# yekaizhou/duet

Hardware: AMD Instinct MI355X
Metric: SV support-read marks clustered+phased /sec; bit-exact phased_sv.vcf vs ref (higher is better)
Workload: dtype u32/u64 integer + f64 threshold compares; 1 GPU; BASELINE configs[1]: synthetic 1 contig, 1001116 SV marks / 100000 candidates / 159991 tagged reads, resident in HBM; step = ef_classify + ef_finalize_own, two launches (phasing, E/F; ef_seed_sort 0: ; marks_per_gpu=1001116, candidates_per_gpu=100000, reads_per_gpu=159991, parallelism=contig-sharded x1, svlen_thres=50, suppread_thres=2, device_preheat_steps=2700

## Files before the change

### duet_amd/csrc/duet_ef.hip

```cpp

#include <hip/hip_runtime.h>
#include <hip/hip_ext.h>
#include <stdint.h>
#include <stdio.h>
#include <stdlib.h>
#include <string.h>
#include <string>
#include <vector>

#include "duet_ef.h"
#include "duet_internal.h"

#pragma clang fp contract(off)

namespace {

#ifdef DUET_STAMPS
#define STAMP(k, i) do { if (threadIdx.x == 0 && p.stamps) p.stamps[((size_t)(k) * 65536 + blockIdx.x) * 8 + (i)] = wall_clock64(); } while (0)
#else
#define STAMP(k, i) do { } while (0)
#endif

#include "duet_seeds.hip.h"

// ... 1397 lines not shown
            uint32_t any = 0;
            for (uint32_t k = k0; k <= k1; ++k) any |= (p.n_one[k] == 0) ? 1u : 0u;
            const uint32_t n0 = p.n_one[k0], base = p.ctg_off[k0] + k0 + 1;
            const bool lds_mode = k0 == k1 && n0 > 0 && n0 <= kOneLds;
            if (lds_mode)
                for (uint32_t i = tid; i < n0; i += 256u) s_one[i] = p.onebuf[base + i];
            __syncthreads();
#pragma unroll
            for (int r = 0; r < TPB; ++r) {
                const uint32_t cc = g0 + 256u * r + tid;
                if (cc < n_cands) finalize_candidate(p, cc, codes[r], pss[r], k0, lds_mode, s_one, n0, any);
            }
            __syncthreads();
            continue;
        }
        const uint32_t c0 = tile * 256u;
        const uint32_t c = c0 + tid;
        const bool live = c < n_cands;
        const uint8_t code = live ? p.out_pred[c] : 0;
        const uint32_t ps_in = live ? p.out_ps[c] : 0;
        if (tid == 0) {
            const uint32_t last = min(c0 + 255u, n_cands - 1);
            const uint32_t k0 = (DYN && p.cand_contig) ? (uint32_t)p.cand_contig[c0] : p.blk_ctg[tile];
            uint32_t k1 = k0;
            while (last >= p.ctg_off[k1 + 1]) ++k1;
            uint32_t any = 0;
            for (uint32_t k = k0; k <= k1; ++k) any |= (p.n_one[k] == 0);
            const uint32_t n0 = p.n_one[k0];
            s_meta[0] = k0;
            s_meta[1] = (k0 == k1 && n0 > 0 && n0 <= kOneLds) ? n0 : kEmpty;
            s_meta[2] = any;
            s_meta[3] = p.ctg_off[k0] + k0 + 1;
        }
        __syncthreads();
        STAMP(2, 1);
        const uint32_t k0 = s_meta[0], n_lds = s_meta[1], any_empty = s_meta[2];
        const bool lds_mode = n_lds != kEmpty;
        if (lds_mode) {
            const uint32_t *src = p.onebuf + s_meta[3];
            for (uint32_t i = tid; i < n_lds; i += 256u) s_one[i] = src[i];
            __syncthreads();
        }
        STAMP(2, 2);
        if (live) finalize_candidate(p, c, code, ps_in, k0, lds_mode, s_one, n_lds, any_empty);
        if (!DYN) break;
        __syncthreads();
    }
}

constexpr uint32_t kOwnMaxTiles = 2048;
constexpr uint32_t kOwnTab = 2048;
constexpr uint32_t kOwnKeys = 1024;

struct OwnArgs {
    TileRecs recs;
    const uint64_t *seed_ent, *read_tag;
    const uint32_t *cand_pos, *cand_off, *cand_svread, *cand_refread, *mark_read, *c2rec;
    uint32_t *out_ps, *status;
    uint8_t *out_pred;
    uint32_t c_lo, c_hi;
};

template <class F>
__device__ __forceinline__ void own_each_entry(TileRecs recs, const uint64_t *seed_ent, uint32_t c_lo, uint32_t c_hi, uint32_t first,
                                               uint32_t stride, F f)
{
    const uint32_t b_lo = c_lo / kCandPerBlock, b_hi = (c_hi - 1) / kCandPerBlock;
    for (uint32_t b = b_lo + first; b <= b_hi; b += stride) {
        const ulonglong4 rec = recs[b];
        const uint32_t cnt = (uint32_t)rec.x;
        for (uint32_t j = 0; j < cnt; ++j) {
            const uint64_t e = j == 0 ? rec.y : (j == 1 ? rec.z : (j == 2 ? rec.w : seed_ent[(size_t)b * kCandPerBlock + j]));
            const uint32_t c = (uint32_t)(e >> 32);
            if (c >= c_lo && c < c_hi) f((uint32_t)e);
        }
    }
}

__device__ __forceinline__ uint32_t own_nearest_walk(const OwnArgs &a, uint32_t pos)
{
    uint32_t best = 0;
    int64_t bd = -1;
    own_each_entry(a.recs, a.seed_ent, a.c_lo, a.c_hi, 0u, 1u, [&](uint32_t ps) {
        const int64_t d = llabs((int64_t)pos - (int64_t)ps);
        if (bd < 0 || d < bd || (d == bd && ps > best)) { bd = d; best = ps; }
    });
    return best;
}
__device__ __forceinline__ bool own_member_walk(const OwnArgs &a, uint32_t key)
{
    bool hit = false;
    own_each_entry(a.recs, a.seed_ent, a.c_lo, a.c_hi, 0u, 1u, [&](uint32_t ps) { hit = hit || ps == key; });
    return hit;
}

template <class F>
__device__ __forceinline__ void own_each_tag(const OwnArgs &a, uint32_t b, uint32_t e, F f)
{
    for (uint32_t m = b; m < e; ++m) {
        const uint32_t r = a.mark_read[m];
        f(r == kEmpty ? kUntagged : a.read_tag[r]);
    }
}

__device__ __forceinline__ void finalize_candidate_walk(const OwnArgs &a, uint32_t c, uint32_t code, uint32_t ps_in)
{
    if (code & kDivZero) {
        atomicOr(&a.status[0], 1u);
        a.out_pred[c] = 0;
        a.out_ps[c] = 0;
        return;
    }
    const uint32_t c_pos = a.cand_pos[c];
    if (code & (kClass2 | kClass2Slow)) {
        Vote v = {0, 0, 0, 0, 0, 0};
        uint32_t ps = 0;
        const uint32_t mb = a.cand_off[c], me = a.cand_off[c + 1];
        if (code & kClass2) {
            const uint32_t *rec = a.c2rec + (size_t)ps_in * kC2Words;
            v.allhap = rec[0];
            const uint32_t ng = rec[1];
            uint32_t best = 0;
            for (uint32_t k = 0; k < (uint32_t)kC2Groups; ++k) {
                const uint32_t *g = rec + 2 + 6 * k;
                if (k < ng && g[1] > best && own_member_walk(a, g[0])) {
                    best = g[1];
                    ps = g[0];
                    v.hap1 = g[2]; v.hap2 = g[3];
                    v.t1 = g[4]; v.t2 = g[5];
                    v.hap0 = v.allhap - v.hap1 - v.hap2;
                }
            }
        } else {
            uint32_t best = 0;
            own_each_tag(a, mb, me, [&](uint64_t t) {
                if (t != kUntagged && tag_pc(t) <= kPcMax) ++v.allhap;
            });
            uint32_t done_ps = kEmpty;
            own_each_tag(a, mb, me, [&](uint64_t t) {
                if (t == kUntagged || tag_pc(t) > kPcMax) return;
                const uint32_t g = tag_ps(t);
                if (g == done_ps || (g == ps && best)) return;
                if (!own_member_walk(a, g)) return;
                uint32_t n = 0, n1 = 0, n2 = 0;
                uint64_t s1 = 0, s2 = 0;
                own_each_tag(a, mb, me, [&](uint64_t u) {
                    if (u == kUntagged || tag_pc(u) > kPcMax || tag_ps(u) != g) return;
                    ++n;
                    const uint32_t hap = tag_hap(u), pc = tag_pc(u);
                    n1 += hap == 1 ? 1u : 0u; s1 += hap == 1 ? pc : 0u;
                    n2 += hap == 2 ? 1u : 0u; s2 += hap == 2 ? pc : 0u;
                });
                done_ps = g;
                if (n > best) {
                    best = n; ps = g;
                    v.hap1 = n1; v.hap2 = n2; v.t1 = s1; v.t2 = s2;
                    v.hap0 = v.allhap - n1 - n2;
                }
            });
        }
        if (v.hap1 == 0 && v.hap2 == 0) ps = own_nearest_walk(a, c_pos);
        a.out_pred[c] = (uint8_t)decide(2, v, me - mb, a.cand_svread[c], a.cand_refread[c]);
        a.out_ps[c] = ps;
        return;
    }
    a.out_pred[c] = (uint8_t)(code & 3u);
    a.out_ps[c] = own_nearest_walk(a, c_pos);
}

__device__ __forceinline__ uint32_t wave_max_u32(uint32_t v)
{
    v = max(v, (uint32_t)__builtin_amdgcn_update_dpp(0, (int)v, 0xB1, 0xF, 0xF, false));
    v = max(v, (uint32_t)__builtin_amdgcn_update_dpp(0, (int)v, 0x4E, 0xF, 0xF, false));
    v = max(v, (uint32_t)__builtin_amdgcn_update_dpp(0, (int)v, 0x124, 0xF, 0xF, false));
    v = max(v, (uint32_t)__builtin_amdgcn_update_dpp(0, (int)v, 0x128, 0xF, 0xF, false));
    v = max(v, (uint32_t)__builtin_amdgcn_update_dpp(0, (int)v, 0x142, 0xA, 0xF, false));
    v = max(v, (uint32_t)__builtin_amdgcn_update_dpp(0, (int)v, 0x143, 0xC, 0xF, false));
    return (uint32_t)__builtin_amdgcn_readlane((int)v, 63);
}

__device__ __forceinline__ void own_sort_set(const uint32_t *s_tab, uint32_t *s_key, uint32_t *s_one, uint32_t *s_part, uint32_t u)
{
    const uint32_t tid = threadIdx.x, lane = tid & 63u, wave = tid >> 6;
    uint32_t mv[kOwnTab / 256u], cnt = 0;
#pragma unroll
    for (uint32_t j = 0; j < kOwnTab / 256u; ++j) {
        mv[j] = s_tab[tid + 256u * j];
        cnt += mv[j] != kEmpty ? 1u : 0u;
    }
    uint32_t x = cnt;
#pragma unroll
    for (int d = 1; d < 64; d <<= 1) {
        const uint32_t y = __shfl_up(x, d, 64);
        if ((int)lane >= d) x += y;
    }
    if (lane == 63) s_part[wave] = x;
    __syncthreads();
    uint32_t at = x - cnt;
#pragma unroll
    for (uint32_t w = 0; w < 4; ++w) at += w < wave ? s_part[w] : 0u;
#pragma unroll
    for (uint32_t j = 0; j < kOwnTab / 256u; ++j)
        if (mv[j] != kEmpty) s_key[at++] = mv[j];
    const uint32_t U = (u + 63u) & ~63u, nblk = U >> 6;
    if (tid < U - u) s_key[u + tid] = kEmpty;
    __syncthreads();
    for (uint32_t b = wave; b < nblk; b += 4u) s_key[b * 64u + lane] = wave_sort64(s_key[b * 64u + lane], lane);
    __syncthreads();
    for (uint32_t i = tid; i < U; i += 256u) {
        const uint32_t me = s_key[i];
        uint32_t rank = 0;
        for (uint32_t b = 0; b < nblk; b += 4u) {
            const uint32_t *b0 = s_key + b * 64u, *b1 = s_key + min(b + 1u, nblk - 1u) * 64u;
            const uint32_t *b2 = s_key + min(b + 2u, nblk - 1u) * 64u, *b3 = s_key + min(b + 3u, nblk - 1u) * 64u;
            uint32_t p0 = 0, p1 = 0, p2 = 0, p3 = 0;
#pragma unroll
            for (uint32_t st = 32; st > 0; st >>= 1) {
                p0 += b0[p0 + st - 1u] < me ? st : 0u;
                p1 += b1[p1 + st - 1u] < me ? st : 0u;
                p2 += b2[p2 + st - 1u] < me ? st : 0u;
                p3 += b3[p3 + st - 1u] < me ? st : 0u;
            }
            p0 += b0[p0] < me ? 1u : 0u;
            p1 += b1[p1] < me ? 1u : 0u;
            p2 += b2[p2] < me ? 1u : 0u;
            p3 += b3[p3] < me ? 1u : 0u;
            rank += p0 + (b + 1u < nblk ? p1 : 0u) + (b + 2u < nblk ? p2 : 0u) + (b + 3u < nblk ? p3 : 0u);
        }
        if (me != kEmpty) s_one[rank] = me;
    }
    __syncthreads();
}

__device__ __forceinline__ void own_vote_from_marks(const uint32_t *mark_read, const uint64_t *read_tag, uint32_t mb, uint32_t me_,
                                                 const uint32_t *s_tab, Vote *vo, uint32_t *pso)
{
    auto each = [&](auto f) {
        for (uint32_t m0 = mb; m0 < me_; m0 += 8) {
            uint32_t r[8];
            uint64_t t[8];
#pragma unroll
            for (int j = 0; j < 8; ++j) r[j] = mark_read[m0 + j < me_ ? m0 + j : mb];
#pragma unroll
            for (int j = 0; j < 8; ++j) t[j] = read_tag[r[j] == kEmpty ? 0u : r[j]];
#pragma unroll
            for (int j = 0; j < 8; ++j)
                if (m0 + j < me_) f(r[j] == kEmpty ? kUntagged : t[j]);
        }
    };
    auto member = [&](uint32_t key) -> bool {
        uint32_t h = (key * 2654435761u) >> (32u - 11u);
        for (;;) {
            const uint32_t v = s_tab[h];
            if (v == key) return true;
            if (v == kEmpty) return false;
            h = (h + 1u) & (kOwnTab - 1u);
        }
    };
    Vote v = {0, 0, 0, 0, 0, 0};
    uint32_t ps = 0, best = 0, done_ps = kEmpty;
    each([&](uint64_t t) {
        if (t != kUntagged && tag_pc(t) <= kPcMax) ++v.allhap;
    });
    each([&](uint64_t t) {
        if (t == kUntagged || tag_pc(t) > kPcMax) return;
        const uint32_t g = tag_ps(t);
        if (g == done_ps || (g == ps && best)) return;
        if (!member(g)) return;
        uint32_t n = 0, n1 = 0, n2 = 0;
        uint64_t s1 = 0, s2 = 0;
        each([&](uint64_t u) {
            if (u == kUntagged || tag_pc(u) > kPcMax || tag_ps(u) != g) return;
            ++n;
            const uint32_t hap = tag_hap(u), pc = tag_pc(u);
            n1 += hap == 1 ? 1u : 0u; s1 += hap == 1 ? pc : 0u;
            n2 += hap == 2 ? 1u : 0u; s2 += hap == 2 ? pc : 0u;
        });
        done_ps = g;
        if (n > best) {
            best = n; ps = g;
            v.hap1 = n1; v.hap2 = n2; v.t1 = s1; v.t2 = s2;
            v.hap0 = v.allhap - n1 - n2;
        }
    });
    *vo = v;
    *pso = ps;
}

__device__ __forceinline__ bool own_probe(uint32_t *s_tab, uint32_t key, uint32_t h)
{
    for (uint32_t probes = 0; probes < kOwnTab; ++probes) {
        const uint32_t old = atomicCAS(&s_tab[h], kEmpty, key);
        if (old == kEmpty) return true;
        if (old == key) return false;
        h = (h + 1u) & (kOwnTab - 1u);
    }
    return false;
}

constexpr uint32_t kOwnWin = 64;

__global__ __launch_bounds__(256) void ef_finalize_own(const Params p)
{
    __shared__ uint32_t s_tab[kOwnTab];
    __shared__ uint32_t s_key[kOwnKeys];
    __shared__ uint32_t s_one[kOwnKeys];
    __shared__ uint32_t s_win[kOwnWin];
    __shared__ uint32_t s_mm[4][2];
    __shared__ uint32_t s_red[4][3];
    __shared__ uint32_t s_part[4];
    __shared__ uint32_t s_nwin;
    __shared__ __align__(8) uint32_t s_c2[kC2Quota * kC2Words];
    const uint32_t tid = threadIdx.x, lane = tid & 63u, wave = tid >> 6;
    STAMP(2, 0);
    if (blockIdx.x == 0 && tid == 0) p.status[1] = 0;
    const uint32_t n_cands = p.C;
    const uint32_t nK = p.n_small;
    auto coff = [&](uint32_t kk) -> uint32_t { return p.ctg_small[kk]; };
    const uint32_t tile = blockIdx.x;
    const uint32_t c0 = tile * 256u, c = c0 + tid;
    const bool live = c < n_cands;
    const uint32_t cl = live ? c : n_cands - 1u;
    const uint32_t last = min(c0 + 255u, n_cands - 1);
    const uint32_t keys_cap = (p.dbg & DUET_DBG_EF_OWN_SMALLTAB) ? 8u : kOwnKeys;
    const uint32_t win_cap = (p.dbg & DUET_DBG_EF_OWN_SMALLTAB) ? 2u : kOwnWin;
    const TileRecs recs{reinterpret_cast<const ulonglong4 *>(p.blk_rec)};
    constexpr uint32_t kPre = 2;
    static_assert(kPre == 2, "the overflow loop selects between rec[0] and rec[1]");
    ulonglong4 rec[kPre], ext[kPre];
    auto load_recs = [&](uint32_t b_lo, uint32_t b_hi) {
#pragma unroll
        for (uint32_t i = 0; i < kPre; ++i) {
            const uint32_t b = min(b_lo + tid + 256u * i, b_hi);
            rec[i] = recs[b];
            ext[i] = recs.second(b);
        }
    };
    const uint32_t code_ld = p.out_pred[cl], ps_ld = p.out_ps[cl], pos_ld = p.cand_pos[cl];
    const uint32_t o0_ld = p.cand_off[cl], o1_ld = p.cand_off[cl + 1u];
    const uint32_t sv_ld = p.cand_svread[cl], rf_ld = p.cand_refread[cl];
    constexpr uint32_t kPairs = kC2Quota * kC2Words / 2;
    const uint2 *c2src = reinterpret_cast<const uint2 *>(p.c2rec + (size_t)tile * kC2Quota * kC2Words);
    const uint2 a0 = c2src[tid], a1 = c2src[tid + 256u < kPairs ? tid + 256u : tid];
    uint32_t lo = 0, hi = nK;
    while (hi - lo > 1) {
        const uint32_t mid = (lo + hi) >> 1;
        if (coff(mid) <= c0) lo = mid; else hi = mid;
    }
    uint32_t k_first = lo;
    while (k_first < nK && coff(k_first) == coff(k_first + 1)) ++k_first;
    {
        const uint32_t kf = k_first < nK ? k_first : 0u;
        load_recs(coff(kf) / kCandPerBlock, (coff(kf + 1) - 1) / kCandPerBlock);
    }
    asm volatile("" ::"v"(code_ld), "v"(ps_ld), "v"(pos_ld), "v"(o0_ld), "v"(o1_ld), "v"(sv_ld), "v"(rf_ld), "v"(a0.x), "v"(a0.y),
                 "v"(a1.x), "v"(a1.y));
    {
        uint2 *dst = reinterpret_cast<uint2 *>(s_c2);
        dst[tid] = a0;
        if (tid + 256u < kPairs) dst[tid + 256u] = a1;
    }
    const uint32_t code = live ? code_ld : 0u, ps_in = live ? ps_ld : 0u, c_pos = live ? pos_ld : 0u;
    const uint32_t c_o0 = live ? o0_ld : 0u, c_o1 = live ? o1_ld : 0u;
    const uint32_t c_svread = live ? sv_ld : 0u, c_refread = live ? rf_ld : 0u;
    for (uint32_t k = lo; k < nK && coff(k) <= last; ++k) {
        const uint32_t c_lo = coff(k), c_hi = coff(k + 1);
        if (c_lo == c_hi) continue;
        const uint32_t b_lo = c_lo / kCandPerBlock, b_hi = (c_hi - 1) / kCandPerBlock;
        if (k != k_first) load_recs(b_lo, b_hi);
#pragma unroll
        for (uint32_t i = 0; i < kOwnTab / 256u; ++i) s_tab[tid + 256u * i] = kEmpty;
        if (tid == 0) s_nwin = 0;
        const bool mine = live && c >= c_lo && c < c_hi;
        const bool asks = mine && code >= 4u && !(code & kDivZero);
        {
            const uint32_t mn = wave_max_u32(asks ? ~c_pos : 0u), mx = wave_max_u32(asks ? c_pos + 1u : 0u);
            if (lane == 0) { s_mm[wave][0] = mn; s_mm[wave][1] = mx; }
        }
        lds_barrier();
        STAMP(2, 1);
        asm volatile("" ::"v"(rec[0].x), "v"(rec[1].x), "v"(rec[0].y), "v"(rec[1].y), "v"(rec[0].z), "v"(rec[1].z), "v"(rec[0].w),
                     "v"(rec[1].w), "v"(ext[0].x), "v"(ext[1].x), "v"(ext[0].y), "v"(ext[1].y), "v"(ext[0].z), "v"(ext[1].z),
                     "v"(ext[0].w), "v"(ext[1].w));
        uint32_t pmin, pmax;
        {
            const uint32_t a0 = max(max(s_mm[0][0], s_mm[1][0]), max(s_mm[2][0], s_mm[3][0]));
            const uint32_t a1 = max(max(s_mm[0][1], s_mm[1][1]), max(s_mm[2][1], s_mm[3][1]));
            pmin = a1 ? ~a0 : 0u;
            pmax = a1 ? a1 - 1u : 0u;
        }
        uint32_t fresh = 0, leftp = 0, rinv = 0;
        static_assert(kOwnTab == 1u << 11, "the hash takes 11 bits");
        auto slot_of = [](uint32_t key) -> uint32_t { return (key * 2654435761u) >> (32u - 11u); };
        auto count_new = [&](bool nw, uint32_t key) {
            fresh += nw ? 1u : 0u;
            leftp = max(leftp, (nw && key <= pmin) ? key + 1u : 0u);
            rinv = max(rinv, (nw && key >= pmax) ? ~key : 0u);
            if (nw && key > pmin && key < pmax) {
                const uint32_t at = atomicAdd(&s_nwin, 1u);
                if (at < kOwnWin) s_win[at] = key;
            }
        };
        auto insert = [&](uint64_t e) {
            const uint32_t cc = (uint32_t)(e >> 32), key = (uint32_t)e;
            if (cc >= c_lo && cc < c_hi) count_new(own_probe(s_tab, key, slot_of(key)), key);
        };
        uint32_t coll = 0;
        auto group = [&](const uint64_t (&e)[4], uint32_t first, uint32_t n_in, uint32_t cnt, uint32_t bit0) {
            uint32_t key[4], old[4];
            bool ok[4];
#pragma unroll
            for (uint32_t j = 0; j < 4; ++j) {
                const uint32_t cc = (uint32_t)(e[j] >> 32);
                key[j] = (uint32_t)e[j];
                ok[j] = j < n_in && first + j < cnt && cc >= c_lo && cc < c_hi;
                old[j] = kEmpty;
            }
#pragma unroll
            for (uint32_t j = 0; j < 4; ++j)
                if (ok[j]) old[j] = atomicCAS(&s_tab[slot_of(key[j])], kEmpty, key[j]);
#pragma unroll
            for (uint32_t j = 0; j < 4; ++j) {
                coll |= (ok[j] && old[j] != kEmpty && old[j] != key[j]) ? 1u << (bit0 + j) : 0u;
                count_new(ok[j] && old[j] == kEmpty, key[j]);
            }
        };
#pragma unroll
        for (uint32_t i = 0; i < kPre; ++i) {
            const uint32_t cnt = b_lo + tid + 256u * i <= b_hi ? (uint32_t)rec[i].x : 0u;
            if (__any(cnt > 0u)) {
                const uint64_t e[4] = {rec[i].y, rec[i].z, rec[i].w, 0ull};
                group(e, 0u, 3u, cnt, 7u * i);
            }
            if (__any(cnt > 3u)) {
                const uint64_t e[4] = {ext[i].x, ext[i].y, ext[i].z, ext[i].w};
                group(e, 3u, 4u, cnt, 7u * i + 3u);
            }
        }
        while (coll) {
            const uint32_t j = (uint32_t)__ffs(coll) - 1u;
            coll &= coll - 1u;
            uint32_t key = 0;
#pragma unroll
            for (uint32_t i = 0; i < kPre; ++i) {
                key = j == 7u * i + 0u ? (uint32_t)rec[i].y : key;
                key = j == 7u * i + 1u ? (uint32_t)rec[i].z : key;
                key = j == 7u * i + 2u ? (uint32_t)rec[i].w : key;
                key = j == 7u * i + 3u ? (uint32_t)ext[i].x : key;
                key = j == 7u * i + 4u ? (uint32_t)ext[i].y : key;
                key = j == 7u * i + 5u ? (uint32_t)ext[i].z : key;
                key = j == 7u * i + 6u ? (uint32_t)ext[i].w : key;
            }
            count_new(own_probe(s_tab, key, (slot_of(key) + 1u) & (kOwnTab - 1u)), key);
        }
        auto overflow = [&](uint32_t b, uint32_t cnt, uint32_t from) {
            constexpr uint32_t kLong = 24;
            if (cnt > from && cnt <= kLong) {
                const uint64_t *ov = p.seed_ent + (size_t)b * kCandPerBlock;
#pragma unroll 1
                for (uint32_t j = from; j < cnt; j += 4) {
                    uint64_t e[4];
#pragma unroll
                    for (uint32_t t = 0; t < 4; ++t) e[t] = ov[min(j + t, cnt - 1u)];
#pragma unroll
                    for (uint32_t t = 0; t < 4; ++t)
                        if (j + t < cnt) insert(e[t]);
                }
            }
            unsigned long long todo = __ballot(cnt > kLong);
            while (todo) {
                const uint32_t h = (uint32_t)__ffsll((long long)todo) - 1u;
                todo &= todo - 1ull;
                const uint32_t b_h = (uint32_t)__builtin_amdgcn_readlane((int)b, h), cnt_h = (uint32_t)__builtin_amdgcn_readlane((int)cnt, h);
                const uint64_t *ov = p.seed_ent + (size_t)b_h * kCandPerBlock;
                for (uint32_t j = from + lane; j < cnt_h; j += 64u) insert(ov[j]);
            }
        };
#pragma unroll 1
        for (uint32_t i = 0, b0 = b_lo; b0 <= b_hi; ++i, b0 += 256u) {
            const uint32_t b = b0 + tid;
            uint32_t cnt, from = 7u;
            if (i < kPre) {
                cnt = b <= b_hi ? (uint32_t)(i == 0 ? rec[0].x : rec[1].x) : 0u;
            } else {
                ulonglong4 r = {0, 0, 0, 0};
                if (b <= b_hi) r = recs[b];
                cnt = (uint32_t)r.x;
                if (cnt > 0) insert(r.y);
                if (cnt > 1) insert(r.z);
                if (cnt > 2) insert(r.w);
                from = 3u;
            }
            overflow(b, cnt, from);
        }
        {
            const uint32_t l = wave_max_u32(leftp), r = wave_max_u32(rinv), o = wave_sum(fresh);
            if (lane == 0) { s_red[wave][0] = l; s_red[wave][1] = r; s_red[wave][2] = o; }
        }
        lds_barrier();
        STAMP(2, 2);
        const uint32_t u = s_red[0][2] + s_red[1][2] + s_red[2][2] + s_red[3][2];
        const uint32_t Lp = max(max(s_red[0][0], s_red[1][0]), max(s_red[2][0], s_red[3][0]));
        const uint32_t Ri = max(max(s_red[0][1], s_red[1][1]), max(s_red[2][1], s_red[3][1]));
        const uint32_t n_win = s_nwin;
        const bool over = u > keys_cap;
        const bool sorted = !over && n_win > win_cap;
        if (sorted) own_sort_set(s_tab, s_key, s_one, s_part, u);
        STAMP(2, 5);
        auto nearest = [&](uint32_t pos) -> uint32_t {
            if (sorted) return nearest_seed(s_one, u, pos);
            uint32_t best = 0;
            int64_t bd = -1;
            auto look = [&](uint32_t v) {
                const int64_t d = llabs((int64_t)pos - (int64_t)v);
                if (bd < 0 || d < bd || (d == bd && v > best)) { bd = d; best = v; }
            };
            if (Lp) look(Lp - 1u);
            if (Ri) look(~Ri);
            for (uint32_t i = 0; i < n_win; ++i) look(s_win[i]);
            return best;
        };
        auto member = [&](uint32_t key) -> bool {
            uint32_t h = (key * 2654435761u) >> (32u - 11u);
            for (;;) {
                const uint32_t v = s_tab[h];
                if (v == key) return true;
                if (v == kEmpty) return false;
                h = (h + 1u) & (kOwnTab - 1u);
            }
        };
        if (mine) {
            if (u == 0) {
                if (code != 0) p.out_pred[c] = 0;
                if (ps_in != 0) p.out_ps[c] = 0;
            } else if (code >= 4u) {
                if (code & kDivZero) {
                    atomicOr(&p.status[0], 1u);
                    p.out_pred[c] = 0;
                    p.out_ps[c] = 0;
                } else if (over) {
                    const OwnArgs a = {recs, p.seed_ent, p.read_tag, p.cand_pos, p.cand_off, p.cand_svread, p.cand_refread, p.mark_read, p.c2rec,
                                       p.out_ps, p.status, p.out_pred, c_lo, c_hi};
                    finalize_candidate_walk(a, c, code, ps_in);
                } else if (code & kClass2Slow) {
                    Vote v;
                    uint32_t ps;
                    own_vote_from_marks(p.mark_read, p.read_tag, c_o0, c_o1, s_tab, &v, &ps);
                    if (v.hap1 == 0 && v.hap2 == 0) ps = nearest(c_pos);
                    p.out_pred[c] = (uint8_t)decide(2, v, c_o1 - c_o0, c_svread, c_refread);
                    p.out_ps[c] = ps;
                } else if (code & kClass2) {
                    uint32_t w[kC2Words];
                    const uint32_t own0 = tile * kC2Quota;
                    if (ps_in >= own0 && ps_in < own0 + kC2Quota) {
#pragma unroll
                        for (int i = 0; i < kC2Words; ++i) w[i] = s_c2[(ps_in - own0) * kC2Words + i];
                    } else {
                        const uint32_t *rec2 = p.c2rec + (size_t)ps_in * kC2Words;
#pragma unroll
                        for (int i = 0; i < kC2Words; ++i) w[i] = rec2[i];
                    }
                    Vote v = {0, 0, 0, 0, 0, 0};
                    uint32_t ps = 0, best = 0;
                    v.allhap = w[0];
                    const uint32_t ng = w[1];
#pragma unroll
                    for (int g = 0; g < kC2Groups; ++g) {
                        if ((uint32_t)g < ng && w[2 + 6 * g + 1] > best && member(w[2 + 6 * g])) {
                            best = w[2 + 6 * g + 1];
                            ps = w[2 + 6 * g];
                            v.hap1 = w[2 + 6 * g + 2]; v.hap2 = w[2 + 6 * g + 3];
                            v.t1 = w[2 + 6 * g + 4]; v.t2 = w[2 + 6 * g + 5];
                            v.hap0 = v.allhap - v.hap1 - v.hap2;
                        }
                    }
                    if (v.hap1 == 0 && v.hap2 == 0) ps = nearest(c_pos);
                    p.out_pred[c] = (uint8_t)decide(2, v, c_o1 - c_o0, c_svread, c_refread);
                    p.out_ps[c] = ps;
                } else {
                    p.out_pred[c] = (uint8_t)(code & 3u);
                    p.out_ps[c] = nearest(c_pos);
                }
            }
        }
        STAMP(2, 6);
        __syncthreads();
    }
}

__global__ void plan_mark_starts(const uint32_t *ctg_off, uint32_t K, uint8_t *ctg_start)
{
    const uint32_t k = blockIdx.x * blockDim.x + threadIdx.x;
    if (k < K && ctg_off[k] < ctg_off[k + 1]) ctg_start[ctg_off[k]] = 1;
}

__global__ void plan_device(const uint32_t *ctg_off, uint32_t K, uint32_t B, uint32_t *ctg_off_copy, uint32_t *n_one_and_status,
                            uint32_t *blk_ctg)
{
    const uint32_t b = blockIdx.x * blockDim.x + threadIdx.x;
    if (b <= K) ctg_off_copy[b] = ctg_off[b];
    if (b < K + 8) n_one_and_status[b] = 0;
    if (b >= B) return;
    const uint32_t c = b * kCandPerBlock;
    uint32_t lo = 0, hi = K;
    while (hi - lo > 1) {
        const uint32_t mid = (lo + hi) >> 1;
        if (ctg_off[mid] <= c) lo = mid; else hi = mid;
    }
    blk_ctg[b] = lo;
}

__global__ void plan_device_contigs(const uint16_t *cand_contig, const uint32_t *n_cands, uint32_t K, uint32_t B,
                                    uint32_t *ctg_off_copy, uint32_t *n_one_and_status, uint32_t *blk_ctg)
{
    const uint32_t t = blockIdx.x * blockDim.x + threadIdx.x;
    const uint32_t N = *n_cands;
    if (t <= K) {
        uint32_t lo = 0, hi = N;
        while (lo < hi) {
            const uint32_t mid = lo + ((hi - lo) >> 1);
            if (cand_contig[mid] < t) lo = mid + 1; else hi = mid;
        }
        ctg_off_copy[t] = t == K ? N : lo;
    }
    if (t < K + 8) n_one_and_status[t] = 0;
    if (t < B) {
        const uint32_t c = t * kCandPerBlock;
        blk_ctg[t] = c < N ? (uint32_t)cand_contig[c] : 0u;
    }
}


}

thread_local std::string duet_g_last_error;

namespace {

inline int fail(duet_ctx *ctx, int code, const std::string &msg) { return duet_fail(ctx, code, msg); }
inline int reserve(duet_ctx *ctx, DevBuf &b, size_t bytes) { return duet_reserve(ctx, b, bytes); }

size_t c2_slots(uint32_t B, uint32_t C) { return (size_t)B * kC2Quota + (C / 8u > 256u ? C / 8u : 256u); }

int ensure_plan(duet_ctx *ctx, const duet_ef_problem *pr, hipStream_t stream)
{
    const uint32_t K = pr->n_contigs, C = pr->n_cands;
    if (ctx->plan_C == C && ctx->plan_off.size() == (size_t)K + 1 && ctx->plan_stream == stream &&
        memcmp(ctx->plan_off.data(), pr->cand_ctg_off, sizeof(uint32_t) * (K + 1)) == 0)
        return DUET_OK;
    const uint32_t B = (C + kCandPerBlock - 1) / kCandPerBlock;
    const size_t small_words = (size_t)(K + 1) + K + 8 + (size_t)B + 16 + (size_t)B * 16;
    const size_t want[6] = {small_words * 4, C, (size_t)B * kCandPerBlock * 8, ((size_t)C + K + 1) * 4, ((size_t)C + K + 1) * 4,
                            c2_slots(B, C) * kC2Words * 4};
    DevBuf *bufs[6] = {&ctx->ws_small, &ctx->ws_start, &ctx->ws_ent, &ctx->ws_one, &ctx->ws_tmp, &ctx->ws_c2};
    bool grow = ctx->plan_stream != stream;
    for (int i = 0; i < 6; ++i) grow = grow || want[i] > bufs[i]->cap;
    const size_t stage_bytes = ((size_t)K + 1 + B) * 4;
    grow = grow || stage_bytes > ctx->plan_stage_cap;
    int rc;
    if (grow) {
        HIP_TRY(ctx, hipDeviceSynchronize());
        for (int i = 0; i < 6; ++i)
            if ((rc = reserve(ctx, *bufs[i], want[i]))) return rc;
        if (stage_bytes > ctx->plan_stage_cap) {
            if (ctx->plan_stage) HIP_TRY(ctx, hipHostFree(ctx->plan_stage));
            ctx->plan_stage = nullptr;
            ctx->plan_stage_cap = 0;
            HIP_TRY(ctx, hipHostMalloc((void **)&ctx->plan_stage, stage_bytes + stage_bytes / 4 + 4096, hipHostMallocDefault));
            ctx->plan_stage_cap = stage_bytes + stage_bytes / 4 + 4096;
        }
    } else {
        HIP_TRY(ctx, hipEventSynchronize(ctx->plan_ev));
    }
    uint32_t *w = (uint32_t *)ctx->ws_small.ptr;
    ctx->d_ctg_off = w;            w += K + 1;
    ctx->d_n_one = w;              w += K;
    ctx->d_status = w;             w += 8;
    ctx->d_blk_ctg = w;            w += B;
    w += ((uintptr_t)w & 63) ? (64 - ((uintptr_t)w & 63)) / 4 : 0;
    ctx->d_blk_cnt = w;
    uint32_t *h_off = ctx->plan_stage, *h_blk = ctx->plan_stage + (K + 1);
    memcpy(h_off, pr->cand_ctg_off, sizeof(uint32_t) * (K + 1));
    {
        uint32_t k = 0;
        for (uint32_t b = 0; b < B; ++b) {
            const uint32_t c = b * kCandPerBlock;
            while (c >= pr->cand_ctg_off[k + 1]) ++k;
            h_blk[b] = k;
        }
    }
    HIP_TRY(ctx, hipMemcpyAsync(ctx->d_ctg_off, h_off, sizeof(uint32_t) * (K + 1), hipMemcpyHostToDevice, stream));
    if (B) HIP_TRY(ctx, hipMemcpyAsync(ctx->d_blk_ctg, h_blk, sizeof(uint32_t) * B, hipMemcpyHostToDevice, stream));
    HIP_TRY(ctx, hipEventRecord(ctx->plan_ev, stream));
    HIP_TRY(ctx, hipMemsetAsync(ctx->d_n_one, 0, sizeof(uint32_t) * ((size_t)K + 8), stream));
    if (C) HIP_TRY(ctx, hipMemsetAsync(ctx->ws_start.ptr, 0, C, stream));
    hipLaunchKernelGGL(plan_mark_starts, dim3((K + 255) / 256), dim3(256), 0, stream, ctx->d_ctg_off, K,
                       (uint8_t *)ctx->ws_start.ptr);
    HIP_TRY(ctx, hipGetLastError());
    ctx->ef_seeds_stale = false;
    ctx->plan_off.assign(pr->cand_ctg_off, pr->cand_ctg_off + K + 1);
    ctx->plan_C = C;
    ctx->plan_stream = stream;
    return DUET_OK;
}

int validate(duet_ctx *ctx, const duet_ef_problem *pr, const void *out_pred, const void *out_ps)
{
    if (!ctx) return fail(nullptr, DUET_ERR_INVALID, "null context");
    if (!pr) return fail(ctx, DUET_ERR_INVALID, "null problem");
    if (!pr->cand_ctg_off) return fail(ctx, DUET_ERR_INVALID, "cand_ctg_off is null");
    if (pr->n_contigs == 0 && pr->n_cands != 0) return fail(ctx, DUET_ERR_INVALID, "candidates without contigs");
    if (pr->cand_ctg_off[0] != 0 || pr->cand_ctg_off[pr->n_contigs] != pr->n_cands)
        return fail(ctx, DUET_ERR_INVALID, "cand_ctg_off must start at 0 and end at n_cands");
    for (uint32_t k = 0; k < pr->n_contigs; ++k)
        if (pr->cand_ctg_off[k] > pr->cand_ctg_off[k + 1])
            return fail(ctx, DUET_ERR_INVALID, "cand_ctg_off must be non-decreasing");
    if (pr->n_cands) {
        if (!pr->cand_pos || !pr->cand_svlen || !pr->cand_svread || !pr->cand_refread || !pr->cand_gt_ok ||
            !pr->cand_off || !pr->mark_read || !out_pred || !out_ps)
            return fail(ctx, DUET_ERR_INVALID, "null array");
        if (pr->n_reads && !pr->read_tag) return fail(ctx, DUET_ERR_INVALID, "read_tag is null");
    }
    return DUET_OK;
}

}

extern "C" {

int duet_abi_version(void) { return DUET_ABI_VERSION; }

const char *duet_last_error(const duet_ctx *ctx) { return ctx ? ctx->err.c_str() : duet_g_last_error.c_str(); }

duet_ctx *duet_ctx_create(int device_id)
{
    int n = 0;
    hipError_t e = hipGetDeviceCount(&n);
    if (e != hipSuccess || n <= 0) {
        duet_g_last_error = std::string("no HIP device: ") + (e != hipSuccess ? hipGetErrorString(e) : "device count is 0");
        return nullptr;
    }
    if (device_id < 0 || device_id >= n) {
        duet_g_last_error = "device id out of range";
        return nullptr;
    }
    if ((e = hipSetDevice(device_id)) != hipSuccess) {
        duet_g_last_error = std::string("hipSetDevice: ") + hipGetErrorString(e);
        return nullptr;
    }
    hipDeviceProp_t prop;
    if ((e = hipGetDeviceProperties(&prop, device_id)) != hipSuccess) {
        duet_g_last_error = std::string("hipGetDeviceProperties: ") + hipGetErrorString(e);
        return nullptr;
    }
    if (strncmp(prop.gcnArchName, "gfx950", 6) != 0) {
        duet_g_last_error = std::string("device is ") + prop.gcnArchName + ", this library is built for gfx950 only";
// ... 404 lines not shown
```

Measured before the change: 63.72 billion marks/s.

## Batch hash-table inserts in finalize_own and aggregate window appends per wave

The kernel now issues all preloaded entries' LDS atomicCAS inserts in one unrolled batch. Non-owned entries go to a per-lane dummy slot instead of being branched around. The left/right boundary bookkeeping becomes min reductions rather than per-entry count_new calls. Per-lane atomicAdd on the window counter is replaced by a wave-level ballot prefix sum with a single atomic per wave, and collision reprobing is skipped unless some lane saw a foreign key. The aim is to cut divergent control flow and LDS atomic contention, at the cost of more registers for the key/old arrays and a slightly larger shared table.

Result: no change. 63.69 billion marks/s, median of 4 (-0.0%).

```diff
diff --git a/duet_amd/csrc/duet_ef.hip b/duet_amd/csrc/duet_ef.hip
--- a/duet_amd/csrc/duet_ef.hip
+++ b/duet_amd/csrc/duet_ef.hip
@@ -1723,7 +1723,7 @@
 
 __global__ __launch_bounds__(256) void ef_finalize_own(const Params p)
 {
-    __shared__ uint32_t s_tab[kOwnTab];
+    __shared__ uint32_t s_tab[kOwnTab + 64];
     __shared__ uint32_t s_key[kOwnKeys];
     __shared__ uint32_t s_one[kOwnKeys];
     __shared__ uint32_t s_win[kOwnWin];
@@ -1791,6 +1791,7 @@
         if (k != k_first) load_recs(b_lo, b_hi);
 #pragma unroll
         for (uint32_t i = 0; i < kOwnTab / 256u; ++i) s_tab[tid + 256u * i] = kEmpty;
+        if (tid < 64u) s_tab[kOwnTab + tid] = kEmpty;
         if (tid == 0) s_nwin = 0;
         const bool mine = live && c >= c_lo && c < c_hi;
         const bool asks = mine && code >= 4u && !(code & kDivZero);
@@ -1803,6 +1804,7 @@
         asm volatile("" ::"v"(rec[0].x), "v"(rec[1].x), "v"(rec[0].y), "v"(rec[1].y), "v"(rec[0].z), "v"(rec[1].z), "v"(rec[0].w),
                      "v"(rec[1].w), "v"(ext[0].x), "v"(ext[1].x), "v"(ext[0].y), "v"(ext[1].y), "v"(ext[0].z), "v"(ext[1].z),
                      "v"(ext[0].w), "v"(ext[1].w));
+        STAMP(2, 3);
         uint32_t pmin, pmax;
         {
             const uint32_t a0 = max(max(s_mm[0][0], s_mm[1][0]), max(s_mm[2][0], s_mm[3][0]));
@@ -1826,53 +1828,89 @@
             const uint32_t cc = (uint32_t)(e >> 32), key = (uint32_t)e;
             if (cc >= c_lo && cc < c_hi) count_new(own_probe(s_tab, key, slot_of(key)), key);
         };
-        uint32_t coll = 0;
-        auto group = [&](const uint64_t (&e)[4], uint32_t first, uint32_t n_in, uint32_t cnt, uint32_t bit0) {
-            uint32_t key[4], old[4];
-            bool ok[4];
-#pragma unroll
-            for (uint32_t j = 0; j < 4; ++j) {
-                const uint32_t cc = (uint32_t)(e[j] >> 32);
-                key[j] = (uint32_t)e[j];
-                ok[j] = j < n_in && first + j < cnt && cc >= c_lo && cc < c_hi;
-                old[j] = kEmpty;
-            }
-#pragma unroll
-            for (uint32_t j = 0; j < 4; ++j)
-                if (ok[j]) old[j] = atomicCAS(&s_tab[slot_of(key[j])], kEmpty, key[j]);
-#pragma unroll
-            for (uint32_t j = 0; j < 4; ++j) {
-                coll |= (ok[j] && old[j] != kEmpty && old[j] != key[j]) ? 1u << (bit0 + j) : 0u;
-                count_new(ok[j] && old[j] == kEmpty, key[j]);
-            }
-        };
+        constexpr uint32_t kEnt = 7u * kPre;
+        const uint32_t n_c = c_hi - c_lo;
+        uint32_t key[kEnt], old[kEnt], left_d = kEmpty, right_d = kEmpty;
+        bool take[kEnt];
 #pragma unroll
         for (uint32_t i = 0; i < kPre; ++i) {
             const uint32_t cnt = b_lo + tid + 256u * i <= b_hi ? (uint32_t)rec[i].x : 0u;
-            if (__any(cnt > 0u)) {
-                const uint64_t e[4] = {rec[i].y, rec[i].z, rec[i].w, 0ull};
-                group(e, 0u, 3u, cnt, 7u * i);
-            }
-            if (__any(cnt > 3u)) {
-                const uint64_t e[4] = {ext[i].x, ext[i].y, ext[i].z, ext[i].w};
-                group(e, 3u, 4u, cnt, 7u * i + 3u);
-            }
-        }
-        while (coll) {
-            const uint32_t j = (uint32_t)__ffs(coll) - 1u;
-            coll &= coll - 1u;
-            uint32_t key = 0;
-#pragma unroll
-            for (uint32_t i = 0; i < kPre; ++i) {
-                key = j == 7u * i + 0u ? (uint32_t)rec[i].y : key;
-                key = j == 7u * i + 1u ? (uint32_t)rec[i].z : key;
-                key = j == 7u * i + 2u ? (uint32_t)rec[i].w : key;
-                key = j == 7u * i + 3u ? (uint32_t)ext[i].x : key;
-                key = j == 7u * i + 4u ? (uint32_t)ext[i].y : key;
-                key = j == 7u * i + 5u ? (uint32_t)ext[i].z : key;
-                key = j == 7u * i + 6u ? (uint32_t)ext[i].w : key;
-            }
-            count_new(own_probe(s_tab, key, (slot_of(key) + 1u) & (kOwnTab - 1u)), key);
+#pragma unroll
+            for (uint32_t j = 0; j < 7; ++j) take[7 * i + j] = __any(cnt > (j < 3u ? 0u : j));
+        }
+        asm volatile("" ::"v"(pmin), "v"(pmax));
+#pragma unroll
+        for (uint32_t i = 0; i < kPre; ++i) {
+            const uint32_t cnt = b_lo + tid + 256u * i <= b_hi ? (uint32_t)rec[i].x : 0u;
+            const uint64_t e[7] = {rec[i].y, rec[i].z, rec[i].w, ext[i].x, ext[i].y, ext[i].z, ext[i].w};
+#pragma unroll
+            for (uint32_t j = 0; j < 7; ++j) {
+                const uint32_t n = 7 * i + j;
+                key[n] = kEmpty;
+                old[n] = kEmpty;
+                if (!take[n]) continue;
+                const bool ok = (j < cnt) & ((uint32_t)(e[j] >> 32) - c_lo < n_c);
+                key[n] = ok ? (uint32_t)e[j] : kEmpty;
+                uint32_t slot = slot_of((uint32_t)e[j]);
+                asm volatile("" : "+v"(slot));
+                old[n] = atomicCAS(&s_tab[ok ? slot : kOwnTab + lane], kEmpty, key[n]);
+                left_d = min(left_d, pmin - key[n]);
+                right_d = min(right_d, key[n] - pmax);
+            }
+        }
+        leftp = max(leftp, left_d <= pmin ? pmin - left_d + 1u : 0u);
+        rinv = max(rinv, right_d <= 0xFFFFFFFEu - pmax ? ~(pmax + right_d) : 0u);
+        const uint32_t width = pmax > pmin ? pmax - pmin - 1u : 0u;
+        uint32_t inwin = 0;
+        uint32_t met_other = 0;
+#pragma unroll
+        for (uint32_t n = 0; n < kEnt; ++n) {
+            if (!take[n]) continue;
+            const bool won = old[n] == kEmpty;
+            const uint32_t mine_new = won ? key[n] : kEmpty;
+            fresh += mine_new != kEmpty ? 1u : 0u;
+            inwin |= mine_new - pmin - 1u < width ? 1u << n : 0u;
+            met_other |= (won ? key[n] : old[n]) ^ key[n];
+        }
+#ifdef DUET_STAMPS
+        asm volatile("" ::"v"(inwin), "v"(met_other), "v"(fresh));
+#endif
+        STAMP(2, 4);
+        if (__builtin_amdgcn_ballot_w64(met_other != 0u) != 0) {
+            uint32_t coll = 0;
+#pragma unroll
+            for (uint32_t n = 0; n < kEnt; ++n)
+                coll |= ((old[n] != kEmpty) & (old[n] != key[n])) ? 1u << n : 0u;
+            while (coll) {
+                const uint32_t j = (uint32_t)__ffs(coll) - 1u;
+                coll &= coll - 1u;
+                uint32_t k1 = 0;
+#pragma unroll
+                for (uint32_t n = 0; n < kEnt; ++n) k1 = j == n ? key[n] : k1;
+                const bool nw = own_probe(s_tab, k1, (slot_of(k1) + 1u) & (kOwnTab - 1u));
+                fresh += nw ? 1u : 0u;
+                inwin |= (nw && k1 > pmin && k1 < pmax) ? 1u << j : 0u;
+            }
+        }
+        if (__builtin_amdgcn_ballot_w64(inwin != 0u) != 0) {
+            const uint32_t mine_n = (uint32_t)__popc(inwin);
+            uint32_t before = 0, total = 0;
+#pragma unroll
+            for (uint32_t b = 0; b < 4; ++b) {
+                const uint64_t m = __builtin_amdgcn_ballot_w64(((mine_n >> b) & 1u) != 0u);
+                before += __builtin_amdgcn_mbcnt_hi((uint32_t)(m >> 32), __builtin_amdgcn_mbcnt_lo((uint32_t)m, 0u)) << b;
+                total += (uint32_t)__popcll(m) << b;
+            }
+            uint32_t at = 0;
+            if (lane == 0) at = atomicAdd(&s_nwin, total);
+            at = (uint32_t)__builtin_amdgcn_readfirstlane((int)at) + before;
+#pragma unroll
+            for (uint32_t n = 0; n < kEnt; ++n) {
+                const bool mine_in = ((inwin >> n) & 1u) != 0u;
+                if (!take[n] || __builtin_amdgcn_ballot_w64(mine_in) == 0) continue;
+                if (mine_in && at < kOwnWin) s_win[at] = key[n];
+                at += mine_in ? 1u : 0u;
+            }
         }
         auto overflow = [&](uint32_t b, uint32_t cnt, uint32_t from) {
             constexpr uint32_t kLong = 24;
```
